# mila-iqia/babyai

Hardware: NVIDIA H100
Metric: env-steps/sec at 65 536 envs (GoToLocal); obs bit-exact vs CPU ref (higher is better)
Workload: dtype u8

## Files before the change

babyai_b200/csrc/env_logic.cuh:

```cuda
#pragma once
#include <stdint.h>

#if defined(__CUDACC__)
#define BB_HD __host__ __device__ __forceinline__
#define BB_HD_NOINLINE __host__ __device__ __noinline__
#define BB_ALIGN16 __align__(16)
#else
#define BB_ALIGN16 alignas(16)
#define BB_HD inline
#define BB_HD_NOINLINE
#endif

#ifndef BB_GEN_COOP
#define BB_GEN_COOP 1
#endif
#if defined(__CUDA_ARCH__) && BB_GEN_COOP
#define BB_GEN_WARP 1
#else
#define BB_GEN_WARP 0
#endif
#ifndef BB_GEN_OUTLINE
#define BB_GEN_OUTLINE 1
#endif
#if defined(__CUDA_ARCH__) && BB_GEN_COOP
// ... 25 lines not shown
constexpr int CELL_EMPTY = T_EMPTY;
constexpr int CELL_WALL = T_WALL | (C_GREY << 3);
constexpr int NO_OBJ = 0xFF;
constexpr int CARRY_UNTRACKED = 0x40;
constexpr int MAXUNTRACKED = 32;
constexpr int MAXOBJ = 32;
constexpr int MAXH = 25;
constexpr int MAXROOMS = 16;
constexpr int MAXTOK = 72;
constexpr int OBS_BYTES = 147;
constexpr int OBS_WORDS = 37;

enum : int {
    W_PAD = 0, W_GO, W_TO, W_PICK, W_UP, W_OPEN, W_PUT, W_NEXT, W_THE, W_A, W_OBJECT,
    W_RED, W_GREEN, W_BLUE, W_PURPLE, W_YELLOW, W_GREY,
    W_BOX, W_BALL, W_KEY, W_DOOR,
    W_IN, W_FRONT, W_OF, W_YOU, W_BEHIND, W_ON, W_YOUR, W_LEFT, W_RIGHT,
    W_THEN, W_AFTER, W_AND, W_COUNT
};

struct LevelParams {
    int32_t kind, room_size, num_rows, num_cols, num_dists, instr, doors_open, grey_dists;
    int32_t locations, unblocking, implicit_unlock;
    int32_t all_unique, require_unreachable;
    int32_t n_action_kinds, action_kinds[4];
    int32_t n_instr_kinds, instr_kinds[3];
    int32_t W, H, cells, cells_pad, max_tokens, nav_time_maze;
    int32_t strict_mask, done_actions;
    int32_t col_mul;
    int32_t kinds_mask, single_instr;
    int32_t bonus, bonus_a, bonus_b;
    int32_t box_contains;
    int32_t obj_words;
    int32_t rs_g, rs_t, gt_off;
    uint64_t locked_thr;
    uint32_t wall_rows[MAXH];
    int32_t small;
    uint64_t wall64;
    uint64_t row_tmpl[16];
};

struct BB_ALIGN16 EnvHot {
    uint8_t x, y;
    uint8_t dirflags;
    uint8_t carry;
    uint16_t step_count, max_steps;
    uint32_t cur_mask;
    uint32_t snap_mask;
};
struct BB_ALIGN16 ObjTab {
    uint8_t x[MAXOBJ], y[MAXOBJ];
    uint8_t tc[MAXOBJ];
};
struct BB_ALIGN16 InstrRec {
    uint32_t desc_mask[8];
    uint8_t leaf_kind[4];
    uint8_t leaf_pre[4];
    uint8_t root_kind;
    uint8_t side_and;
    uint8_t flags;
    uint8_t pad0;
    uint32_t pad1;
};
struct BB_ALIGN16 RngRec { uint64_t seed, draws; };

BB_HD uint32_t mulhi32(uint32_t a, uint32_t b)
// ... 2087 lines not shown
```

babyai_b200/csrc/level_params.h:

```cpp
#pragma once
#include <math.h>
#include <string.h>
#include "../../include/babyai_b200.h"
#include "env_logic.cuh"

namespace bb {

static inline const char *make_level_params(const bb_level_spec *s, LevelParams *lp)
{
    memset(lp, 0, sizeof *lp);
    if (s->kind < 0 || s->kind > 5) return "bad level kind";
    if (s->kind == BB_KIND_BONUS) { if (s->room_size < 3 || s->room_size > 20 || s->bonus < 1 || s->bonus > 20) return "bad bonus level"; }
    else if (s->room_size < 4 || s->room_size > 8) return "room_size must be in 4..8";
    if (s->num_rows < 1 || s->num_cols < 1 || s->num_rows * s->num_cols > MAXROOMS) return "too many rooms";
    lp->kind = s->kind; lp->room_size = s->room_size; lp->num_rows = s->num_rows; lp->num_cols = s->num_cols;
    lp->num_dists = s->num_dists; lp->instr = s->instr; lp->doors_open = s->doors_open; lp->grey_dists = s->grey_dists;
    lp->locations = s->locations; lp->unblocking = s->unblocking; lp->implicit_unlock = s->implicit_unlock;
    lp->all_unique = s->all_unique; lp->require_unreachable = s->require_unreachable;
    lp->strict_mask = s->strict_mask & 0x1F; lp->done_actions = s->done_actions ? 1 : 0;
    lp->kinds_mask = 0xF; lp->single_instr = 1;
    if (s->kind == BB_KIND_REDBALL || s->kind == BB_KIND_IMPUNLOCK) lp->kinds_mask = 1 << BB_I_GOTO;
    else if (s->kind == BB_KIND_OBJ) lp->kinds_mask = 1 << s->instr;
    else if (s->kind == BB_KIND_UNLOCK) lp->kinds_mask = 1 << BB_I_OPEN;
    else if (s->kind == BB_KIND_LEVELGEN) {
        lp->kinds_mask = 0;
        for (int i = 0; i < s->n_action_kinds && i < 4; i++) lp->kinds_mask |= 1 << s->action_kinds[i];
        lp->single_instr = s->n_instr_kinds == 1 && s->instr_kinds[0] == BB_K_ACTION;
    } else if (s->kind == BB_KIND_BONUS) lp->single_instr = !(s->bonus == 14 || s->bonus == 19 || s->bonus == 20);
    lp->bonus = s->kind == BB_KIND_BONUS ? s->bonus : 0; lp->bonus_a = s->bonus_a; lp->bonus_b = s->bonus_b;
    lp->box_contains = lp->bonus == BN_KEY_IN_BOX ? 2 : 0;
    if (s->kind == BB_KIND_OBJ && (s->instr < BB_I_GOTO || s->instr > BB_I_PUTNEXT)) return "bad instruction kind";
    if (s->kind == BB_KIND_OBJ && s->instr == BB_I_PUTNEXT && s->num_dists < 2) return "PutNext needs two objects";
    lp->n_action_kinds = s->n_action_kinds; lp->n_instr_kinds = s->n_instr_kinds;
    for (int i = 0; i < 4; i++) lp->action_kinds[i] = s->action_kinds[i];
    for (int i = 0; i < 3; i++) lp->instr_kinds[i] = s->instr_kinds[i];
    lp->col_mul = s->num_cols > 0 ? (64 + s->num_cols - 1) / s->num_cols : 64;
    for (int r = 0; r < s->num_rows * s->num_cols; r++)
        if (s->num_cols <= 0 || ((r * lp->col_mul) >> 6) != r / s->num_cols) return "unsupported room grid (room / num_cols by multiplication)";
    lp->W = (s->room_size - 1) * s->num_cols + 1;
    lp->H = (s->room_size - 1) * s->num_rows + 1;
    if (lp->W > MAXH || lp->H > MAXH) return "grid too large";
    lp->cells = lp->W * lp->H;
    lp->rs_g = (lp->W + 3) / 4 * 4;
    lp->rs_t = (lp->H + 3) / 4 * 4;
    lp->gt_off = (lp->H * lp->rs_g + 15) / 16 * 16;
    lp->cells_pad = lp->gt_off + (lp->W * lp->rs_t + 15) / 16 * 16;
    lp->nav_time_maze = s->room_size * s->room_size * s->num_rows * s->num_cols;
    int max_objs = s->num_dists + (s->kind == BB_KIND_OBJ ? 0 : 1);
    if (s->kind == BB_KIND_IMPUNLOCK) {
        if (s->num_rows * s->num_cols < 2) return "GoToImpUnlock needs at least two rooms";
        max_objs = s->num_dists * (s->num_rows * s->num_cols - 1) + 2;
    }
    if (s->kind == BB_KIND_UNLOCK) {
        if (s->num_rows * s->num_cols < 2) return "Unlock needs at least two rooms";
        if (s->num_dists * (s->num_rows * s->num_cols - 1) + 1 > MAXUNTRACKED) return "too many untracked objects";
        max_objs = 0;
    }
    if (s->kind == BB_KIND_LEVELGEN) {
        if (s->n_action_kinds < 1 || s->n_action_kinds > 4 || s->n_instr_kinds < 1 || s->n_instr_kinds > 3)
            return "bad LevelGen kinds";
        double t = ceil(s->locked_room_prob * 4294967296.0);
// ... 51 lines not shown
```

babyai_b200/csrc/pool.cu:

```cuda
#include <cuda_runtime.h>
#include <stdint.h>
#include <stdio.h>
#include <string.h>
#include <math.h>
#include <new>
#include <vector>
#include <stdlib.h>

#include "../../include/babyai_b200.h"
#include "env_logic.cuh"
#include "level_params.h"
#include "simt.cuh"
#include "gen_round.cuh"
#include "rollout_lane.cuh"
#include "rollout_cta.cuh"
#include "step8.cuh"
#include <type_traits>
#include "rgb_tiles.h"

using namespace bb;

struct PoolPtrs {
    uint8_t *grid; EnvHot *hot; ObjTab *obj; InstrRec *ins; int16_t *tok;
    uint8_t *rgrid; EnvHot *rhot; ObjTab *robj; InstrRec *rins; int16_t *rtok;
// ... 77 lines not shown
        const uint32_t mneed = __ballot_sync(FULL, need);
        if (mneed) {
            uint32_t base = 0;
            if (lane == 0) base = atomicAdd(P.gen_ticket, (uint32_t)__popc(mneed));
            base = __shfl_sync(FULL, base, 0);
            if (need) {
                uint32_t idx = base + (uint32_t)__popc(mneed & ((1u << lane) - 1u));
                if (idx < count) {
                    int b = 3;
                    if (idx >= c3) { idx -= c3; b = 2; if (idx >= c2) { idx -= c2; b = 1; if (idx >= c1) { idx -= c1; b = 0; } } }
                    env = P.gen_list[(size_t)b * P.n + idx];
                    tl = P.tail[env];
                    left = target - (int)(tl - P.head_snap[env]);
                    const RngRec r = P.rng[env];
                    ds.init(&s_ring[0][tid], GS_THREADS, r.seed, r.draws);
                } else exhausted = true;
            }
        }
        const bool active = left > 0;
        const uint32_t mact = __ballot_sync(FULL, active);
        if (!mact) break;
        const bool low = __any_sync(FULL, active && target - left < min_keep);
        if (max_rounds > 0 && rounds >= max_rounds && !low) break;
        if (min_active > 0 && rounds >= 1 && __popc(mact) < min_active && !low && !__any_sync(FULL, active && left > (int)(D / 2))) break;
        rounds++;
        gen_small_round<DrawRing, false>(lp, P, ds, active, env, tl, left, D);
    }
}

constexpr int R_WARPS = 2;
constexpr int R_THREADS = 32 * R_WARPS;
constexpr int R_THREADS_FUSED = R_THREADS + 32;

struct SmemOnlyMem {
    const LevelParams &lp; uint8_t *g, *o, *i;
    __device__ __forceinline__ SmemOnlyMem(const LevelParams &lp_, uint8_t *g_, uint8_t *o_, uint8_t *i_) : lp(lp_), g(g_), o(o_), i(i_) {}
    __device__ __forceinline__ int cell(int x, int y) const { return g[y * lp.rs_g + x]; }
    __device__ __forceinline__ void set_cell(int x, int y, int v) { bb::set_cell(lp, g, x, y, v); }
    __device__ __forceinline__ uint32_t word_at(int off) const { return *reinterpret_cast<const uint32_t *>(g + off); }
    __device__ __forceinline__ int ox(int k) const { return o[k]; }
    __device__ __forceinline__ int oy(int k) const { return o[MAXOBJ + k]; }
    __device__ __forceinline__ int otc(int k) const { return o[2 * MAXOBJ + k]; }
    __device__ __forceinline__ uint32_t oxw(int i) const { return reinterpret_cast<const uint32_t *>(o)[i]; }
    __device__ __forceinline__ uint32_t oyw(int i) const { return reinterpret_cast<const uint32_t *>(o)[MAXOBJ / 4 + i]; }
    __device__ __forceinline__ void set_oxy(int k, int x, int y) { o[k] = (uint8_t)x; o[MAXOBJ + k] = (uint8_t)y; }
    __device__ __forceinline__ uint32_t desc_mask(int d) const { return reinterpret_cast<const uint32_t *>(i)[d]; }
    __device__ __forceinline__ int leaf_kind(int l) const { return i[32 + l]; }
    __device__ __forceinline__ int leaf_pre(int l) const { return i[36 + l]; }
    __device__ __forceinline__ void set_leaf_pre(int l, int v) { i[36 + l] = (uint8_t)v; }
    __device__ __forceinline__ int root_kind() const { return i[40]; }
    __device__ __forceinline__ int side_and() const { return i[41]; }
    __device__ __forceinline__ void set_side_and(int v) { i[41] = (uint8_t)v; }
    __device__ __forceinline__ int flags() const { return i[42]; }
    __device__ __forceinline__ void set_flags(int v) { i[42] = (uint8_t)v; }
    __device__ __forceinline__ int start_carry() const { return i[43]; }
};

template <int K>
struct SmemRoomKindMem : SmemOnlyMem {
    static constexpr int spec_room_kinds = K;
    __device__ __forceinline__ SmemRoomKindMem(const LevelParams &lp_, uint8_t *g_, uint8_t *o_, uint8_t *i_) : SmemOnlyMem(lp_, g_, o_, i_) {}
};

template <int ACT_BYTES, bool UNTR = false, int ROOM_KINDS = 0>
__global__ void __launch_bounds__(R_THREADS_FUSED, 7)
k_rollout(const LevelParams lp, const PoolPtrs P, const void *__restrict__ actions_v, uint8_t *__restrict__ obs,
          float *__restrict__ reward, uint8_t *__restrict__ done, int8_t *__restrict__ dirs, const int n, const int T,
          const int mode, const int force_reset, const int gen_rounds, const int gen_min_active)
{
    extern __shared__ __align__(16) uint32_t smr[];
    const int lane = threadIdx.x & 31, warp = threadIdx.x >> 5;
    const int warp_words = rl_warp_words(lp);
    const bool fused = gen_rounds > 0;
    uint32_t *g_area = smr + R_WARPS * warp_words;
    volatile int *s_done = reinterpret_cast<volatile int *>(g_area + RG_AREA_WORDS - 4);
    if (warp == R_WARPS) {
        rollout_gen_warp(lp, P, g_area, s_done, n, T, blockIdx.x * R_WARPS * 32, gen_rounds, gen_min_active, lane, R_WARPS);
        return;
    }
    rollout_lane_step_warp<PoolPtrs, typename std::conditional<ROOM_KINDS != 0, SmemRoomKindMem<ROOM_KINDS>, SmemOnlyMem>::type, ACT_BYTES, UNTR>(lp, P, actions_v, obs, reward, done, dirs, n, T, mode, force_reset, fused,
                                                                   smr + warp * warp_words, lane, blockIdx.x * R_WARPS + warp, s_done);
}

template <bool UNTR>
__global__ void __launch_bounds__(RC_THREADS, 7)
k_rollout_cta(const LevelParams lp, const PoolPtrs P, const int8_t *__restrict__ actions, uint8_t *__restrict__ obs,
              float *__restrict__ reward, uint8_t *__restrict__ done, int8_t *__restrict__ dirs, const int n, const int T, const int mode)
{
    extern __shared__ __align__(16) uint32_t smc[];
    rollout_cta_role<PoolPtrs, UNTR>(lp, P, actions, obs, reward, done, dirs, n, T, mode, smc, threadIdx.x, blockIdx.x);
}
#if BB_GEN_COOP
template <bool IMPUNLOCK>
__global__ void __launch_bounds__(GEN_THREADS)
k_gen(const LevelParams lp, const PoolPtrs P, const int n, const int target, const int lanes_per_warp, const int chain_cap)
{
    __shared__ typename GenMemFor<IMPUNLOCK>::type gen_mem[GEN_THREADS / 32];
    GenMem *mem = &gen_mem[threadIdx.x >> 5];
    const int lane = threadIdx.x & 31;
    const uint32_t c3 = P.gen_count[3], c2 = P.gen_count[2], c1 = P.gen_count[1], c0 = P.gen_count[0];
    const uint32_t count = c0 + c1 + c2 + c3;
    const uint32_t D = (uint32_t)P.depth;
    for (;;) {
        uint32_t idx = 0;
        if (lane == 0) idx = atomicAdd(P.gen_ticket, 1u);
        idx = __shfl_sync(0xFFFFFFFFu, idx, 0);
        if (idx >= count) break;
        int b = 3;
        if (idx >= c3) { idx -= c3; b = 2; if (idx >= c2) { idx -= c2; b = 1; if (idx >= c1) { idx -= c1; b = 0; } } }
        const int env = P.gen_list[(size_t)b * n + idx];
        const uint32_t t0 = P.tail[env];
        const int have = (int)(t0 - P.head_snap[env]);
        int m = target - have;
// ... 483 lines not shown
    cudaStream_t st = (cudaStream_t)stream;
    if (sched_leave_rollout(p, st)) return 1;
    if (sched_before_step(p, p->rel, st)) return 1;
    launch_step(p, actions_dev, action_bytes, obs_dev, reward_dev, done_dev, dir_dev, 0, st);
    if (sched_after_step(p, p->rel, st)) return 1;
    p->rel++;
    CU(cudaGetLastError());
    return 0;
}

int bb_pool_step_timed(bb_pool *p, const void *actions_dev, int32_t action_bytes, uint8_t *obs_dev, float *reward_dev,
                       uint8_t *done_dev, int8_t *dir_dev, float *ms_step, float *ms_gen)
{
    if (!p || !actions_dev || !obs_dev || !reward_dev || !done_dev || !ms_step || !ms_gen) return fail("bad arguments");
    CU(cudaSetDevice(p->device));
    if (!p->ev[0]) for (int i = 0; i < 3; i++) CU(cudaEventCreate(&p->ev[i]));
    if (sched_join(p, p->stream)) return 1;
    p->after_rollout = false;
    launch_gen(p, p->stream);
    CU(cudaEventRecord(p->ev[0], p->stream));
    launch_step(p, actions_dev, action_bytes, obs_dev, reward_dev, done_dev, dir_dev, 0, p->stream);
    CU(cudaEventRecord(p->ev[1], p->stream));
    launch_gen(p, p->stream);
    CU(cudaEventRecord(p->ev[2], p->stream));
    CU(cudaEventSynchronize(p->ev[2]));
    CU(cudaEventElapsedTime(ms_step, p->ev[0], p->ev[1]));
    CU(cudaEventElapsedTime(ms_gen, p->ev[1], p->ev[2]));
    return 0;
}

static int rollout_graph(bb_pool *p, const int8_t *actions_dev, int32_t T, uint8_t *obs_dev, float *reward_dev,
                         uint8_t *done_dev, int8_t *dir_dev, cudaStream_t user);

int bb_pool_rollout(bb_pool *p, const int8_t *actions_dev, int32_t T, uint8_t *obs_dev, float *reward_dev,
                    uint8_t *done_dev, int8_t *dir_dev, void *stream)
{
    if (!p || !actions_dev || !obs_dev || !reward_dev || !done_dev || T < 1) return fail("bad arguments");
    BB_CHECK_RINGS(p);
    CU(cudaSetDevice(p->device));
    cudaStream_t user = (cudaStream_t)stream;
    const bool conc = p->gen_concurrent && p->mode == BB_MODE_AUTORESET;
    const bool kgen_levels = !(p->lp.small && !p->gen_generic);
    const int cap = kgen_levels && p->chain_cap > 0 && p->D >= 4 * T ? p->chain_cap : 0;
    int R = p->refill_every;
    if (conc) R = p->D / (2 * T);
    if (cap) R = p->D / (4 * T);
    if (conc || cap) { if (R > 8) R = 8; if (p->refill_cap > 0 && R > p->refill_cap) R = p->refill_cap; }
    const bool persistent = p->lp.cells_pad <= p->persist_max_cells && !p->no_persistent &&
                            (p->mode == BB_MODE_FREEZE || (conc || cap ? R >= 1 : p->D >= (p->refill_every + 1) * T));
    if (!persistent) return rollout_graph(p, actions_dev, T, obs_dev, reward_dev, done_dev, dir_dev, user);
    if (T != p->last_T) { p->rollouts = 0; p->last_T = T; }
    const bool refill_slot = (p->rollouts % R) == 0;
    if (!conc || refill_slot) { if (sched_join(p, user)) return 1; }
    const size_t smem = (size_t)R_WARPS * rl_warp_words(p->lp) * 4;
    const int blocks = (p->n + 32 * R_WARPS - 1) / (32 * R_WARPS);
    const bool fused = !p->rollout_cta && p->gen_fused != 0 && (p->gen_fused == 2 || 3 * p->lp.nav_time_maze >= 2 * T) &&
                       p->lp.small && !p->gen_generic && !p->gen_concurrent && p->mode == BB_MODE_AUTORESET &&
                       p->D >= 2 * T + 8 && !getenv("BB_DEBUG_NO_REFILL");
    if (fused && T > p->fused_T) launch_gen(p, user);
    p->fused_T = fused ? T : 0;
    const bool refill = !fused && p->mode == BB_MODE_AUTORESET && !getenv("BB_DEBUG_NO_REFILL") && refill_slot;
    p->rollouts++;
    const bool dbg_timing = p->time_rollout;
    cudaEvent_t *dbg_ev = p->tev;
    if (dbg_timing && !dbg_ev[0]) for (int i = 0; i < 4; i++) CU(cudaEventCreate(&dbg_ev[i]));
    const size_t nb = (size_t)p->n * sizeof(uint32_t);
    const bool gen_serial = !p->gen_concurrent;
    if (refill && gen_serial) {
        if (dbg_timing) cudaEventRecord(dbg_ev[2], user);
        const bool fused_snap = p->lp.small && !p->gen_generic;
        if (!fused_snap) CU(cudaMemcpyAsync(p->P.head_snap, p->P.head, nb, cudaMemcpyDeviceToDevice, user));
        launch_gen_kernel(p, p->D, user, p->gen_budget, p->gen_min_active, fused_snap, p->refill_every * T, false, cap);
        cudaMemcpyAsync(p->P.tail_pub, p->P.tail, nb, cudaMemcpyDeviceToDevice, user);
        if (dbg_timing) { cudaEventRecord(dbg_ev[3], user); p->tev_refill = true; }
        p->launches++;
    } else if (refill) {
        CU(cudaMemcpyAsync(p->P.head_snap, p->P.head, nb, cudaMemcpyDeviceToDevice, user));
        CU(cudaEventRecord(p->ev_fork, user));
    }
    if (dbg_timing) cudaEventRecord(dbg_ev[0], user);
    if (p->rollout_cta) {
        const int blocks_c = (p->n + RC_ENVS - 1) / RC_ENVS;
        const size_t smc = (size_t)rc2_cta_words(p->lp) * 4;
        if (p->lp.kind == KIND_UNLOCK) k_rollout_cta<true><<<blocks_c, RC_THREADS, smc, user>>>(p->lp, p->P, actions_dev, obs_dev, reward_dev, done_dev, dir_dev, p->n, T, p->mode);
        else k_rollout_cta<false><<<blocks_c, RC_THREADS, smc, user>>>(p->lp, p->P, actions_dev, obs_dev, reward_dev, done_dev, dir_dev, p->n, T, p->mode);
    }
    else {
        const int gr = fused ? (p->gen_budget > 0 ? p->gen_budget : 1 << 20) : 0, gm = fused ? p->gen_min_active : 0;
        const int threads = fused ? R_THREADS_FUSED : R_THREADS;
        const size_t sm = fused ? smem + RG_AREA_WORDS * 4 : smem;
#define BB_LAUNCH_ROLLOUT(...) k_rollout<__VA_ARGS__><<<blocks, threads, sm, user>>>(p->lp, p->P, actions_dev, obs_dev, reward_dev, done_dev, dir_dev, p->n, T, p->mode, 0, gr, gm)
        if (p->lp.kind == KIND_UNLOCK) BB_LAUNCH_ROLLOUT(1, true);
        else if (p->room_kinds == (1 << I_GOTO)) BB_LAUNCH_ROLLOUT(1, false, 1 << I_GOTO);
        else if (p->room_kinds == (1 << I_PICKUP)) BB_LAUNCH_ROLLOUT(1, false, 1 << I_PICKUP);
        else BB_LAUNCH_ROLLOUT(1);
#undef BB_LAUNCH_ROLLOUT
    }
    if (dbg_timing) { cudaEventRecord(dbg_ev[1], user); p->tev_kernel = true; }
    p->launches++;
    if (refill && !gen_serial) {
        CU(cudaStreamWaitEvent(p->gen_stream, p->ev_fork, 0));
        if (dbg_timing) cudaEventRecord(dbg_ev[2], p->gen_stream);
        launch_gen_kernel(p, p->D, p->gen_stream, p->gen_budget, p->gen_min_active, false, (p->refill_every + 1) * T, true, cap);
        cudaMemcpyAsync(p->P.tail_pub, p->P.tail, nb, cudaMemcpyDeviceToDevice, p->gen_stream);
        if (dbg_timing) { cudaEventRecord(dbg_ev[3], p->gen_stream); p->tev_refill = true; }
        p->gen_outstanding = true;
        p->launches++;
    }
    p->rel = 0;
    p->after_rollout = true;
    CU(cudaGetLastError());
    return 0;
}

int bb_pool_rollout_timed(bb_pool *p, const int8_t *actions_dev, int32_t T, uint8_t *obs_dev, float *reward_dev,
                          uint8_t *done_dev, int8_t *dir_dev, float *ms_rollout_kernel, float *ms_refill)
{
    if (!p || !ms_rollout_kernel || !ms_refill) return fail("bad arguments");
    *ms_rollout_kernel = 0; *ms_refill = 0;
    p->time_rollout = true; p->tev_kernel = false; p->tev_refill = false;
    const int rc = bb_pool_rollout(p, actions_dev, T, obs_dev, reward_dev, done_dev, dir_dev, p->stream);
    p->time_rollout = false;
    if (rc) return rc;
    CU(cudaStreamSynchronize(p->stream));
    CU(cudaDeviceSynchronize());
    if (p->tev[0] && p->tev_kernel) {
        CU(cudaEventElapsedTime(ms_rollout_kernel, p->tev[0], p->tev[1]));
        if (p->tev_refill) CU(cudaEventElapsedTime(ms_refill, p->tev[2], p->tev[3]));
    }
    return 0;
}

static int rollout_graph(bb_pool *p, const int8_t *actions_dev, int32_t T, uint8_t *obs_dev, float *reward_dev,
                         uint8_t *done_dev, int8_t *dir_dev, cudaStream_t user)
{
    GraphKey key = { actions_dev, obs_dev, reward_dev, done_dev, dir_dev, T, p->mode };
    if (!p->graph || memcmp(&key, &p->gkey, sizeof key) != 0) {
        if (p->graph) { cudaGraphExecDestroy(p->graph); p->graph = nullptr; }
        cudaGraph_t g;
        const size_t n = (size_t)p->n;
        const long long l0 = p->launches;
        const bool saved_out = p->gen_outstanding;
        CU(cudaStreamBeginCapture(p->stream, cudaStreamCaptureModeThreadLocal));
        p->gen_outstanding = false;
// ... 213 lines not shown
```

babyai_b200/csrc/rollout_lane.cuh:

```cuda
#pragma once
#include "simt.cuh"

namespace bb {

constexpr int RL_OBJ_STRIDE = 25, RL_INS_STRIDE = 13;
constexpr int RL_TILE_WORDS = 32 * OBS_BYTES / 4;
constexpr int R_STEP_WARPS = 2;

BB_HD int rl_warp_words(const LevelParams &lp) { return 32 * (((lp.cells_pad >> 2) | 1) + RL_OBJ_STRIDE + RL_INS_STRIDE) + RL_TILE_WORDS; }

template <bool TO_SMEM>
BB_DEV void rl_copy_records(uint32_t *sm, int stride_words, uint4 *glob, int chunks_per_env, int nv, int lane)
{
    for (int idx = lane; idx < nv * chunks_per_env; idx += 32) {
        const int e = idx / chunks_per_env, w0 = (idx - e * chunks_per_env) * 4;
        uint32_t *d = sm + e * stride_words + w0;
        if (TO_SMEM) { const uint4 v = glob[idx]; d[0] = v.x; d[1] = v.y; d[2] = v.z; d[3] = v.w; }
        else glob[idx] = make_uint4(d[0], d[1], d[2], d[3]);
    }
}

BB_DEV void rl_store_tile_plain(const uint32_t *tile, uint8_t *dst, int lane, int valid_envs)
{
    const uint8_t *s = reinterpret_cast<const uint8_t *>(tile);
    const int nbytes = valid_envs * OBS_BYTES;
    for (int i = lane; i < nbytes; i += 32) dst[i] = s[i];
}

template <class PP, class MemT, int ACT_BYTES, bool UNTR>
BB_DEV void rollout_lane_step_warp(const LevelParams &lp, const PP &P, const void *actions_v, uint8_t *obs, float *reward, uint8_t *done,
                                   int8_t *dirs, const int n, const int T, const int mode, const int force_reset, const bool fused,
                                   uint32_t *warp_smem, const int lane, const int warp_global, volatile int *s_done)
{
    const int8_t *actions = reinterpret_cast<const int8_t *>(actions_v);
    const int gs = (lp.cells_pad >> 2) | 1;
    const int env0 = warp_global * 32, env = env0 + lane;
    int nv = n - env0; nv = nv > 32 ? 32 : (nv < 0 ? 0 : nv);
    const bool valid = lane < nv;
    uint32_t *sg = warp_smem, *so = sg + 32 * gs, *si = so + 32 * RL_OBJ_STRIDE;
    uint32_t *tile = si + 32 * RL_INS_STRIDE;
    rl_copy_records<true>(sg, gs, reinterpret_cast<uint4 *>(P.grid + (size_t)env0 * lp.cells_pad), lp.cells_pad >> 4, nv, lane);
    rl_copy_records<true>(so, RL_OBJ_STRIDE, reinterpret_cast<uint4 *>(P.obj + env0), 6, nv, lane);
    rl_copy_records<true>(si, RL_INS_STRIDE, reinterpret_cast<uint4 *>(P.ins + env0), 3, nv, lane);
    EnvHot h;
    { uint4 z = make_uint4(0, 0, 0, 0); h = *reinterpret_cast<EnvHot *>(&z); }
    uint32_t head = 0, avail = 0;
    float last_rew = 0.0f;
    if (valid) {
        h = P.hot[env];
        head = P.head[env];
        avail = (fused ? P.tail[env] : BB_LDCG(P.tail_pub + env)) - head;
        if (mode == BB_MODE_FREEZE) last_rew = P.last_reward[env];
    }
    if (fused) BB_ROLE_SYNC(32 * (R_STEP_WARPS + 1));
    BB_SYNCWARP();
    MemT mem(lp, reinterpret_cast<uint8_t *>(sg + lane * gs), reinterpret_cast<uint8_t *>(so + lane * RL_OBJ_STRIDE),
             reinterpret_cast<uint8_t *>(si + lane * RL_INS_STRIDE));
    uint32_t n_step = 0, n_end = 0, n_succ = 0, n_err = 0, consumed = 0;
    const int gchunks = lp.cells_pad >> 4, tchunks = lp.max_tokens >> 3;
    const int rec_chunks = gchunks + 6 + 3;
    bool bulk_pending = false;
    int a_next = 0;
    if (valid && !force_reset) {
        if (ACT_BYTES == 1) a_next = BB_LD_S8(actions + env);
        else a_next = (int)reinterpret_cast<const long long *>(actions_v)[env];
    }
    for (int t = 0; t < T; t++) {
        const int a = a_next;
        if (ACT_BYTES == 1 && valid && t + 1 < T) a_next = BB_LD_S8(actions + (size_t)(t + 1) * n + env);
        float rew = 0.0f; bool dn = false, begin = false;
        if (valid) {
            begin = force_reset != 0;
            if (force_reset) {
            } else if (!(h.dirflags & 4)) {
                const StepResult sr = step_env<UNTR>(h, mem, a);
                rew = sr.reward; dn = sr.done;
                n_step++; n_end += dn; n_succ += sr.success;
                if (dn) {
                    if (mode == BB_MODE_AUTORESET) begin = true;
                    else { h.dirflags |= 4; last_rew = rew; }
                }
            } else { rew = last_rew; dn = true; }
            if (begin && !(consumed < avail && avail <= (uint32_t)P.depth)) { begin = false; n_err++; *P.err_flag = 1; }
        }
        uint32_t mbeg = BB_BALLOT(begin);
        if (mbeg) {
            const uint32_t my_slot = (head + consumed) % (uint32_t)P.depth;
            BB_SYNCWARP();
            while (mbeg) {
                const int src = ffs32(mbeg);
                mbeg &= mbeg - 1;
                const int slot = (int)BB_SHFL(my_slot, src);
                const int e = env0 + src;
                const LevelOut o = r2_ring_slot(lp, P, e, slot);
                for (int c = lane; c < rec_chunks + tchunks; c += 32) {
                    if (c < rec_chunks) {
                        const uint4 *sp; uint32_t *dp; int k = c;
                        if (k < gchunks) { sp = reinterpret_cast<const uint4 *>(o.grid) + k; dp = sg + src * gs + 4 * k; }
                        else if ((k -= gchunks) < 6) { sp = reinterpret_cast<const uint4 *>(o.obj) + k; dp = so + src * RL_OBJ_STRIDE + 4 * k; }
                        else { k -= 6; sp = reinterpret_cast<const uint4 *>(o.ins) + k; dp = si + src * RL_INS_STRIDE + 4 * k; }
                        const uint4 v = BB_LDCG(sp);
                        dp[0] = v.x; dp[1] = v.y; dp[2] = v.z; dp[3] = v.w;
                    } else {
                        const int k = c - rec_chunks;
                        reinterpret_cast<uint4 *>(P.tok + (size_t)e * lp.max_tokens)[k] = BB_LDCG(reinterpret_cast<const uint4 *>(o.tok) + k);
                    }
                }
                if (lane == src) {
                    const uint4 hv = BB_LDCG(reinterpret_cast<const uint4 *>(o.hot));
                    h = *reinterpret_cast<const EnvHot *>(&hv);
                    consumed++;
                }
            }
            BB_SYNCWARP();
        }
        uint32_t w[OBS_WORDS];
#pragma unroll
        for (int k = 0; k < OBS_WORDS; k++) w[k] = 0;
        if (valid) {
            if (mode == BB_MODE_AUTORESET && (int)h.step_count + 2 == (int)h.max_steps && consumed < avail) {
                const LevelOut o = r2_ring_slot(lp, P, env, (int)((head + consumed) % (uint32_t)P.depth));
                BB_PREFETCH_L2(o.grid);
                BB_PREFETCH_L2(o.obj);
                BB_PREFETCH_L2(reinterpret_cast<const uint8_t *>(o.obj) + 64);
                BB_PREFETCH_L2(o.ins);
                BB_PREFETCH_L2(reinterpret_cast<const uint8_t *>(o.ins) + 32);
                BB_PREFETCH_L2(o.hot);
                BB_PREFETCH_L2(o.tok);
            }
            observe(lp, mem, h.x, h.y, h.dirflags & 3, carry_cell_of<UNTR>(h, mem), w);
            const size_t oi = (size_t)t * n + env;
            if (reward) reward[oi] = rew;
            if (done) done[oi] = dn ? 1 : 0;
            if (dirs) dirs[oi] = (int8_t)(h.dirflags & 3);
        }
        if (lane == 0 && bulk_pending) BB_BULK_WAIT_READ();
        bulk_pending = false;
        BB_SYNCWARP();
        {
            const uint32_t next_w0 = BB_SHFL_DOWN(w[0], 1);
            stage_obs_words(tile, w, lane, next_w0);
        }
        uint8_t *dst = obs + ((size_t)t * n + env0) * OBS_BYTES;
        const bool bulk = nv == 32 && (((uintptr_t)dst) & 15) == 0;
        if (bulk) BB_FENCE_ASYNC_SMEM();
        BB_SYNCWARP();
        if (bulk) {
            if (lane == 0) { BB_BULK_STORE(dst, tile, 32 * OBS_BYTES); bulk_pending = true; }
        } else if (nv > 0) {
            rl_store_tile_plain(tile, dst, lane, nv);
            BB_SYNCWARP();
        }
    }
    if (lane == 0 && bulk_pending) BB_BULK_WAIT_READ();
    BB_SYNCWARP();
    rl_copy_records<false>(sg, gs, reinterpret_cast<uint4 *>(P.grid + (size_t)env0 * lp.cells_pad), lp.cells_pad >> 4, nv, lane);
    rl_copy_records<false>(so, RL_OBJ_STRIDE, reinterpret_cast<uint4 *>(P.obj + env0), 6, nv, lane);
    rl_copy_records<false>(si, RL_INS_STRIDE, reinterpret_cast<uint4 *>(P.ins + env0), 3, nv, lane);
    if (valid) {
        P.hot[env] = h;
        P.head[env] = head + consumed;
        if (mode == BB_MODE_FREEZE) P.last_reward[env] = last_rew;
    }
    for (int off = 16; off; off >>= 1) {
        n_step += BB_SHFL_DOWN(n_step, off); n_end += BB_SHFL_DOWN(n_end, off);
        n_succ += BB_SHFL_DOWN(n_succ, off); n_err += BB_SHFL_DOWN(n_err, off);
    }
    if (fused && lane == 0) BB_ATOMIC_ADD(const_cast<int *>(s_done), 1);
    if (lane == 0) {
        unsigned long long *c = P.warp_counters + 4ull * warp_global;
        if (n_step) BB_ATOMIC_ADD(c + 0, (unsigned long long)n_step);
        if (n_end) BB_ATOMIC_ADD(c + 1, (unsigned long long)n_end);
        if (n_succ) BB_ATOMIC_ADD(c + 2, (unsigned long long)n_succ);
        if (n_err) BB_ATOMIC_ADD(c + 3, (unsigned long long)n_err);
    }
}

}
```

babyai_b200/lib.py:

```python
import ctypes as C
import os

from .levels import LevelSpec

HERE = os.path.dirname(os.path.abspath(__file__))
LIB_PATH = os.path.join(HERE, 'libbabyai_b200.so')

SYMBOLS = [
    'bb_pool_create', 'bb_pool_destroy', 'bb_pool_seed', 'bb_pool_set_mode', 'bb_pool_reset', 'bb_pool_step',
    'bb_pool_step_timed', 'bb_pool_rollout', 'bb_pool_rollout_timed', 'bb_pool_step_host', 'bb_pool_reset_host', 'bb_pool_step_learner', 'bb_pool_mission_tokens', 'bb_pool_render_rgb', 'bb_rgb_tiles', 'bb_vocab_size',
    'bb_vocab_word', 'bb_pool_get_state', 'bb_pool_width', 'bb_pool_height', 'bb_pool_num_envs',
    'bb_pool_counters', 'bb_pool_launches', 'bb_last_error',
]

_lib = None


def load():
    global _lib
    if _lib is not None:
        return _lib
    if not os.path.exists(LIB_PATH):
        raise ImportError('%s is missing: the CUDA extension has not been built (python -m babyai_b200.build). '
                          'babyai_b200 has no CPU fallback.' % LIB_PATH)
    L = C.CDLL(LIB_PATH)
    vp, i32, i64 = C.c_void_p, C.c_int32, C.c_int64
    L.bb_pool_create.argtypes = [C.POINTER(LevelSpec), i32, i32, C.POINTER(vp)]
    L.bb_pool_destroy.argtypes = [vp]
    L.bb_pool_seed.argtypes = [vp, vp]
    L.bb_pool_set_mode.argtypes = [vp, i32]
    L.bb_pool_reset.argtypes = [vp, vp, vp, vp]
    L.bb_pool_step.argtypes = [vp, vp, i32, vp, vp, vp, vp, vp]
    L.bb_pool_step_timed.argtypes = [vp, vp, i32, vp, vp, vp, vp, C.POINTER(C.c_float), C.POINTER(C.c_float)]
    L.bb_pool_rollout.argtypes = [vp, vp, i32, vp, vp, vp, vp, vp]
    L.bb_pool_rollout_timed.argtypes = [vp, vp, i32, vp, vp, vp, vp, C.POINTER(C.c_float), C.POINTER(C.c_float)]
    L.bb_pool_step_host.argtypes = [vp, vp, vp, vp, vp, vp]
    L.bb_pool_reset_host.argtypes = [vp, vp, vp]
    L.bb_pool_step_learner.argtypes = [vp, vp, vp, vp, vp, vp, vp]
    L.bb_pool_render_rgb.argtypes = [vp, vp, vp, i32, vp]
    L.bb_rgb_tiles.argtypes = [vp]
    L.bb_pool_mission_tokens.argtypes = [vp, C.POINTER(vp), C.POINTER(i32)]
    L.bb_vocab_size.restype = i32
    L.bb_vocab_word.restype = C.c_char_p
    L.bb_vocab_word.argtypes = [i32]
    L.bb_pool_get_state.argtypes = [vp, i32, vp, vp]
    L.bb_pool_width.argtypes = [vp]
    L.bb_pool_height.argtypes = [vp]
    L.bb_pool_num_envs.argtypes = [vp]
    L.bb_pool_counters.argtypes = [vp, vp]
    L.bb_pool_launches.restype = i64
    L.bb_pool_launches.argtypes = [vp]
    L.bb_last_error.restype = C.c_char_p
    _lib = L
    return L


def check(rc):
    if rc != 0:
        raise RuntimeError('babyai_b200: ' + load().bb_last_error().decode())
```

include/babyai_b200.h:

```cpp
#ifndef BABYAI_B200_H
#define BABYAI_B200_H

#include <stdint.h>

#ifdef __cplusplus
extern "C" {
#endif

#define BB_OBS_BYTES 147
#define BB_MAX_OBJ 32
#define BB_MAX_TOKENS 72

#define BB_KIND_REDBALL 0
#define BB_KIND_OBJ 1
#define BB_KIND_LEVELGEN 2
#define BB_KIND_IMPUNLOCK 3
#define BB_KIND_UNLOCK 4
#define BB_KIND_BONUS 5
#define BB_I_GOTO 0
#define BB_I_PICKUP 1
#define BB_I_OPEN 2
#define BB_I_PUTNEXT 3
#define BB_K_ACTION 0
#define BB_K_AND 1
// ... 14 lines not shown
    int32_t strict_mask;
    int32_t done_actions;
    int32_t bonus, bonus_a, bonus_b;
} bb_level_spec;

typedef struct bb_pool bb_pool;

#define BB_MODE_AUTORESET 0
#define BB_MODE_FREEZE 1

int bb_pool_create(const bb_level_spec *spec, int32_t n_envs, int32_t device, bb_pool **out);
int bb_pool_destroy(bb_pool *pool);

int bb_pool_seed(bb_pool *pool, const uint64_t *seeds_host);

int bb_pool_set_mode(bb_pool *pool, int32_t mode);

int bb_pool_reset(bb_pool *pool, uint8_t *obs_dev, int8_t *dir_dev, void *stream);

int bb_pool_step(bb_pool *pool, const void *actions_dev, int32_t action_bytes,
                 uint8_t *obs_dev, float *reward_dev, uint8_t *done_dev, int8_t *dir_dev, void *stream);

int bb_pool_step_timed(bb_pool *pool, const void *actions_dev, int32_t action_bytes,
                       uint8_t *obs_dev, float *reward_dev, uint8_t *done_dev, int8_t *dir_dev,
                       float *ms_step_kernel, float *ms_gen_kernel);

int bb_pool_rollout(bb_pool *pool, const int8_t *actions_dev, int32_t T,
                    uint8_t *obs_dev, float *reward_dev, uint8_t *done_dev, int8_t *dir_dev, void *stream);

int bb_pool_rollout_timed(bb_pool *pool, const int8_t *actions_dev, int32_t T,
                          uint8_t *obs_dev, float *reward_dev, uint8_t *done_dev, int8_t *dir_dev,
                          float *ms_rollout_kernel, float *ms_refill);

int bb_pool_step_host(bb_pool *pool, const int8_t *actions_host,
                      uint8_t *obs_host, float *reward_host, uint8_t *done_host, int8_t *dir_host);
int bb_pool_reset_host(bb_pool *pool, uint8_t *obs_host, int8_t *dir_host);

int bb_pool_step_learner(bb_pool *pool, const int8_t *actions_host, uint8_t *obs_dev, float *reward_host,
                         uint8_t *done_host, int8_t *dir_dev, void *stream);

int bb_pool_render_rgb(bb_pool *pool, const uint8_t *obs_dev, uint8_t *rgb_dev, int32_t n_obs, void *stream);
int bb_rgb_tiles(uint8_t *tiles_host);

int bb_pool_mission_tokens(bb_pool *pool, const int16_t **tokens_dev, int32_t *max_len);
int32_t bb_vocab_size(void);
const char *bb_vocab_word(int32_t id);

int bb_pool_get_state(bb_pool *pool, int32_t env, uint8_t *grid_host, int32_t *info_host);
int32_t bb_pool_width(const bb_pool *pool);
int32_t bb_pool_height(const bb_pool *pool);
int32_t bb_pool_num_envs(const bb_pool *pool);

int bb_pool_counters(bb_pool *pool, int64_t *out4_host);

int64_t bb_pool_launches(const bb_pool *pool);

const char *bb_last_error(void);

#ifdef __cplusplus
}
#endif
#endif
```

Before: 7.574 billion.

## Pack per-lane object and instruction records compactly in shared memory

Replaces the fixed-stride object and instruction shared-memory tables with one compact per-lane record. Its size follows the level's object count and description words, and objects are laid out interleaved. This shrinks rollout shared memory per warp, and the launch bound is raised from 7 to 8 blocks per SM to use the freed space. For room-kind-specialised kernels it also ignores force_reset, and it adds a query that reports occupancy. The cost is more complex gather/scatter index math when copying records and refilling slots.

```diff
diff --git a/babyai_b200/csrc/env_logic.cuh b/babyai_b200/csrc/env_logic.cuh
--- a/babyai_b200/csrc/env_logic.cuh
+++ b/babyai_b200/csrc/env_logic.cuh
@@ -81,6 +81,7 @@
     int32_t bonus, bonus_a, bonus_b;
     int32_t box_contains;
     int32_t obj_words;
+    int32_t desc_words;
     int32_t rs_g, rs_t, gt_off;
     uint64_t locked_thr;
     uint32_t wall_rows[MAXH];
diff --git a/babyai_b200/csrc/level_params.h b/babyai_b200/csrc/level_params.h
--- a/babyai_b200/csrc/level_params.h
+++ b/babyai_b200/csrc/level_params.h
@@ -27,6 +27,7 @@
         for (int i = 0; i < s->n_action_kinds && i < 4; i++) lp->kinds_mask |= 1 << s->action_kinds[i];
         lp->single_instr = s->n_instr_kinds == 1 && s->instr_kinds[0] == BB_K_ACTION;
     } else if (s->kind == BB_KIND_BONUS) lp->single_instr = !(s->bonus == 14 || s->bonus == 19 || s->bonus == 20);
+    lp->desc_words = lp->single_instr ? 2 : 8;
     lp->bonus = s->kind == BB_KIND_BONUS ? s->bonus : 0; lp->bonus_a = s->bonus_a; lp->bonus_b = s->bonus_b;
     lp->box_contains = lp->bonus == BN_KEY_IN_BOX ? 2 : 0;
     if (s->kind == BB_KIND_OBJ && (s->instr < BB_I_GOTO || s->instr > BB_I_PUTNEXT)) return "bad instruction kind";
diff --git a/babyai_b200/csrc/pool.cu b/babyai_b200/csrc/pool.cu
--- a/babyai_b200/csrc/pool.cu
+++ b/babyai_b200/csrc/pool.cu
@@ -133,38 +133,8 @@
 constexpr int R_THREADS = 32 * R_WARPS;
 constexpr int R_THREADS_FUSED = R_THREADS + 32;
 
-struct SmemOnlyMem {
-    const LevelParams &lp; uint8_t *g, *o, *i;
-    __device__ __forceinline__ SmemOnlyMem(const LevelParams &lp_, uint8_t *g_, uint8_t *o_, uint8_t *i_) : lp(lp_), g(g_), o(o_), i(i_) {}
-    __device__ __forceinline__ int cell(int x, int y) const { return g[y * lp.rs_g + x]; }
-    __device__ __forceinline__ void set_cell(int x, int y, int v) { bb::set_cell(lp, g, x, y, v); }
-    __device__ __forceinline__ uint32_t word_at(int off) const { return *reinterpret_cast<const uint32_t *>(g + off); }
-    __device__ __forceinline__ int ox(int k) const { return o[k]; }
-    __device__ __forceinline__ int oy(int k) const { return o[MAXOBJ + k]; }
-    __device__ __forceinline__ int otc(int k) const { return o[2 * MAXOBJ + k]; }
-    __device__ __forceinline__ uint32_t oxw(int i) const { return reinterpret_cast<const uint32_t *>(o)[i]; }
-    __device__ __forceinline__ uint32_t oyw(int i) const { return reinterpret_cast<const uint32_t *>(o)[MAXOBJ / 4 + i]; }
-    __device__ __forceinline__ void set_oxy(int k, int x, int y) { o[k] = (uint8_t)x; o[MAXOBJ + k] = (uint8_t)y; }
-    __device__ __forceinline__ uint32_t desc_mask(int d) const { return reinterpret_cast<const uint32_t *>(i)[d]; }
-    __device__ __forceinline__ int leaf_kind(int l) const { return i[32 + l]; }
-    __device__ __forceinline__ int leaf_pre(int l) const { return i[36 + l]; }
-    __device__ __forceinline__ void set_leaf_pre(int l, int v) { i[36 + l] = (uint8_t)v; }
-    __device__ __forceinline__ int root_kind() const { return i[40]; }
-    __device__ __forceinline__ int side_and() const { return i[41]; }
-    __device__ __forceinline__ void set_side_and(int v) { i[41] = (uint8_t)v; }
-    __device__ __forceinline__ int flags() const { return i[42]; }
-    __device__ __forceinline__ void set_flags(int v) { i[42] = (uint8_t)v; }
-    __device__ __forceinline__ int start_carry() const { return i[43]; }
-};
-
-template <int K>
-struct SmemRoomKindMem : SmemOnlyMem {
-    static constexpr int spec_room_kinds = K;
-    __device__ __forceinline__ SmemRoomKindMem(const LevelParams &lp_, uint8_t *g_, uint8_t *o_, uint8_t *i_) : SmemOnlyMem(lp_, g_, o_, i_) {}
-};
-
 template <int ACT_BYTES, bool UNTR = false, int ROOM_KINDS = 0>
-__global__ void __launch_bounds__(R_THREADS_FUSED, 7)
+__global__ void __launch_bounds__(R_THREADS_FUSED, 8)
 k_rollout(const LevelParams lp, const PoolPtrs P, const void *__restrict__ actions_v, uint8_t *__restrict__ obs,
           float *__restrict__ reward, uint8_t *__restrict__ done, int8_t *__restrict__ dirs, const int n, const int T,
           const int mode, const int force_reset, const int gen_rounds, const int gen_min_active)
@@ -179,7 +149,7 @@
         rollout_gen_warp(lp, P, g_area, s_done, n, T, blockIdx.x * R_WARPS * 32, gen_rounds, gen_min_active, lane, R_WARPS);
         return;
     }
-    rollout_lane_step_warp<PoolPtrs, typename std::conditional<ROOM_KINDS != 0, SmemRoomKindMem<ROOM_KINDS>, SmemOnlyMem>::type, ACT_BYTES, UNTR>(lp, P, actions_v, obs, reward, done, dirs, n, T, mode, force_reset, fused,
+    rollout_lane_step_warp<PoolPtrs, LaneRecMem<ROOM_KINDS>, ACT_BYTES, UNTR>(lp, P, actions_v, obs, reward, done, dirs, n, T, mode, ROOM_KINDS != 0 ? 0 : force_reset, fused,
                                                                    smr + warp * warp_words, lane, blockIdx.x * R_WARPS + warp, s_done);
 }
 
@@ -729,6 +699,22 @@
 static int rollout_graph(bb_pool *p, const int8_t *actions_dev, int32_t T, uint8_t *obs_dev, float *reward_dev,
                          uint8_t *done_dev, int8_t *dir_dev, cudaStream_t user);
 
+static bool rollout_fused(const bb_pool *p, int T)
+{
+    return !p->rollout_cta && p->gen_fused != 0 && (p->gen_fused == 2 || 3 * p->lp.nav_time_maze >= 2 * T) &&
+           p->lp.small && !p->gen_generic && !p->gen_concurrent && p->mode == BB_MODE_AUTORESET &&
+           p->D >= 2 * T + 8 && !getenv("BB_DEBUG_NO_REFILL");
+}
+
+using RolloutKernel = decltype(&k_rollout<1>);
+static RolloutKernel rollout_kernel(const bb_pool *p)
+{
+    if (p->lp.kind == KIND_UNLOCK) return k_rollout<1, true>;
+    if (p->room_kinds == (1 << I_GOTO)) return k_rollout<1, false, 1 << I_GOTO>;
+    if (p->room_kinds == (1 << I_PICKUP)) return k_rollout<1, false, 1 << I_PICKUP>;
+    return k_rollout<1>;
+}
+
 int bb_pool_rollout(bb_pool *p, const int8_t *actions_dev, int32_t T, uint8_t *obs_dev, float *reward_dev,
                     uint8_t *done_dev, int8_t *dir_dev, void *stream)
 {
@@ -751,9 +737,7 @@
     if (!conc || refill_slot) { if (sched_join(p, user)) return 1; }
     const size_t smem = (size_t)R_WARPS * rl_warp_words(p->lp) * 4;
     const int blocks = (p->n + 32 * R_WARPS - 1) / (32 * R_WARPS);
-    const bool fused = !p->rollout_cta && p->gen_fused != 0 && (p->gen_fused == 2 || 3 * p->lp.nav_time_maze >= 2 * T) &&
-                       p->lp.small && !p->gen_generic && !p->gen_concurrent && p->mode == BB_MODE_AUTORESET &&
-                       p->D >= 2 * T + 8 && !getenv("BB_DEBUG_NO_REFILL");
+    const bool fused = rollout_fused(p, T);
     if (fused && T > p->fused_T) launch_gen(p, user);
     p->fused_T = fused ? T : 0;
     const bool refill = !fused && p->mode == BB_MODE_AUTORESET && !getenv("BB_DEBUG_NO_REFILL") && refill_slot;
@@ -786,12 +770,7 @@
         const int gr = fused ? (p->gen_budget > 0 ? p->gen_budget : 1 << 20) : 0, gm = fused ? p->gen_min_active : 0;
         const int threads = fused ? R_THREADS_FUSED : R_THREADS;
         const size_t sm = fused ? smem + RG_AREA_WORDS * 4 : smem;
-#define BB_LAUNCH_ROLLOUT(...) k_rollout<__VA_ARGS__><<<blocks, threads, sm, user>>>(p->lp, p->P, actions_dev, obs_dev, reward_dev, done_dev, dir_dev, p->n, T, p->mode, 0, gr, gm)
-        if (p->lp.kind == KIND_UNLOCK) BB_LAUNCH_ROLLOUT(1, true);
-        else if (p->room_kinds == (1 << I_GOTO)) BB_LAUNCH_ROLLOUT(1, false, 1 << I_GOTO);
-        else if (p->room_kinds == (1 << I_PICKUP)) BB_LAUNCH_ROLLOUT(1, false, 1 << I_PICKUP);
-        else BB_LAUNCH_ROLLOUT(1);
-#undef BB_LAUNCH_ROLLOUT
+        rollout_kernel(p)<<<blocks, threads, sm, user>>>(p->lp, p->P, actions_dev, obs_dev, reward_dev, done_dev, dir_dev, p->n, T, p->mode, 0, gr, gm);
     }
     if (dbg_timing) { cudaEventRecord(dbg_ev[1], user); p->tev_kernel = true; }
     p->launches++;
@@ -807,6 +786,28 @@
     p->rel = 0;
     p->after_rollout = true;
     CU(cudaGetLastError());
+    return 0;
+}
+
+int bb_pool_rollout_residency(bb_pool *p, int32_t T, int32_t *ctas_per_sm, int32_t *ctas, int32_t *sms)
+{
+    if (!p || T < 1 || !ctas_per_sm || !ctas || !sms) return fail("bad arguments");
+    CU(cudaSetDevice(p->device));
+    const void *fn; int threads; size_t smem;
+    if (p->rollout_cta) {
+        fn = p->lp.kind == KIND_UNLOCK ? (const void *)k_rollout_cta<true> : (const void *)k_rollout_cta<false>;
+        threads = RC_THREADS; smem = (size_t)rc2_cta_words(p->lp) * 4;
+        *ctas = (p->n + RC_ENVS - 1) / RC_ENVS;
+    } else {
+        const bool fused = rollout_fused(p, T);
+        fn = (const void *)rollout_kernel(p);
+        threads = fused ? R_THREADS_FUSED : R_THREADS;
+        smem = (size_t)R_WARPS * rl_warp_words(p->lp) * 4 + (fused ? RG_AREA_WORDS * 4 : 0);
+        *ctas = (p->n + 32 * R_WARPS - 1) / (32 * R_WARPS);
+    }
+    int per_sm = 0;
+    CU(cudaOccupancyMaxActiveBlocksPerMultiprocessor(&per_sm, fn, threads, smem));
+    *ctas_per_sm = per_sm; *sms = p->sm_count;
     return 0;
 }
 
diff --git a/babyai_b200/csrc/rollout_lane.cuh b/babyai_b200/csrc/rollout_lane.cuh
--- a/babyai_b200/csrc/rollout_lane.cuh
+++ b/babyai_b200/csrc/rollout_lane.cuh
@@ -3,11 +3,56 @@
 
 namespace bb {
 
-constexpr int RL_OBJ_STRIDE = 25, RL_INS_STRIDE = 13;
 constexpr int RL_TILE_WORDS = 32 * OBS_BYTES / 4;
 constexpr int R_STEP_WARPS = 2;
 
-BB_HD int rl_warp_words(const LevelParams &lp) { return 32 * (((lp.cells_pad >> 2) | 1) + RL_OBJ_STRIDE + RL_INS_STRIDE) + RL_TILE_WORDS; }
+BB_HD int rl_rec_words(const LevelParams &lp) { return 4 + 3 * lp.obj_words + lp.desc_words; }
+BB_HD int rl_rec_stride(const LevelParams &lp) { return rl_rec_words(lp) | 1; }
+BB_HD int rl_obj_byte(int k) { return 16 + k + ((k >> 2) << 3); }
+BB_HD int rl_mask_byte(const LevelParams &lp, int d) { return 16 + 12 * lp.obj_words + 4 * d; }
+constexpr int RL_CHUNKS = (int)(sizeof(ObjTab) + sizeof(InstrRec)) / 16;
+BB_HD int rl_chunk_word(const LevelParams &lp, int c, int q)
+{
+    if (c < 6) { const int w = 4 * c + q, g = w & 7; return g < lp.obj_words ? 4 + 3 * g + (w >> 3) : -1; }
+    const int w = 4 * (c - 6) + q;
+    return w >= 8 ? w - 8 : (w < lp.desc_words ? 4 + 3 * lp.obj_words + w : -1);
+}
+BB_HD uint32_t *rl_rec_src(const LevelParams &lp, ObjTab *obj, InstrRec *ins, int j)
+{
+    uint32_t *o = reinterpret_cast<uint32_t *>(obj), *i = reinterpret_cast<uint32_t *>(ins);
+    const int ow = 3 * lp.obj_words;
+    if (j < 4) return i + 8 + j;
+    if ((j -= 4) < ow) return o + (j % 3) * (MAXOBJ / 4) + j / 3;
+    return i + (j - ow);
+}
+
+template <int K>
+struct LaneRecMem {
+    static constexpr int spec_room_kinds = K;
+    const LevelParams &lp; uint8_t *g, *r;
+    BB_HD LaneRecMem(const LevelParams &lp_, uint8_t *g_, uint8_t *r_) : lp(lp_), g(g_), r(r_) {}
+    BB_HD int cell(int x, int y) const { return g[y * lp.rs_g + x]; }
+    BB_HD void set_cell(int x, int y, int v) { bb::set_cell(lp, g, x, y, v); }
+    BB_HD uint32_t word_at(int off) const { return load_u32_any(g + off); }
+    BB_HD int ox(int k) const { return r[rl_obj_byte(k)]; }
+    BB_HD int oy(int k) const { return r[rl_obj_byte(k) + 4]; }
+    BB_HD int otc(int k) const { return r[rl_obj_byte(k) + 8]; }
+    BB_HD uint32_t oxw(int i) const { return load_u32_any(r + rl_obj_byte(4 * i)); }
+    BB_HD uint32_t oyw(int i) const { return load_u32_any(r + rl_obj_byte(4 * i) + 4); }
+    BB_HD void set_oxy(int k, int x, int y) { r[rl_obj_byte(k)] = (uint8_t)x; r[rl_obj_byte(k) + 4] = (uint8_t)y; }
+    BB_HD uint32_t desc_mask(int d) const { return load_u32_any(r + rl_mask_byte(lp, d)); }
+    BB_HD int leaf_kind(int l) const { return r[l]; }
+    BB_HD int leaf_pre(int l) const { return r[4 + l]; }
+    BB_HD void set_leaf_pre(int l, int v) { r[4 + l] = (uint8_t)v; }
+    BB_HD int root_kind() const { return r[8]; }
+    BB_HD int side_and() const { return r[9]; }
+    BB_HD void set_side_and(int v) { r[9] = (uint8_t)v; }
+    BB_HD int flags() const { return r[10]; }
+    BB_HD void set_flags(int v) { r[10] = (uint8_t)v; }
+    BB_HD int start_carry() const { return r[11]; }
+};
+
+BB_HD int rl_warp_words(const LevelParams &lp) { return 32 * (((lp.cells_pad >> 2) | 1) + rl_rec_stride(lp)) + RL_TILE_WORDS; }
 
 template <bool TO_SMEM>
 BB_DEV void rl_copy_records(uint32_t *sm, int stride_words, uint4 *glob, int chunks_per_env, int nv, int lane)
@@ -20,6 +65,36 @@
     }
 }
 
+template <bool TO_SMEM>
+BB_DEV void rl_copy_recs(const LevelParams &lp, uint32_t *sr, int rs, ObjTab *obj, InstrRec *ins, int nv, int lane)
+{
+    constexpr int EPP = 32 / RL_CHUNKS;
+    const int c = lane % RL_CHUNKS;
+    int r[4];
+#pragma unroll
+    for (int q = 0; q < 4; q++) r[q] = rl_chunk_word(lp, c, q);
+    if (lane >= EPP * RL_CHUNKS || r[0] < 0) return;
+#pragma unroll 4
+    for (int e = lane / RL_CHUNKS; e < nv; e += EPP) {
+        uint32_t *rec = sr + e * rs;
+        uint4 *g = c < 6 ? reinterpret_cast<uint4 *>(obj + e) + c : reinterpret_cast<uint4 *>(ins + e) + (c - 6);
+        if (TO_SMEM) {
+            const uint4 v = *g;
+            rec[r[0]] = v.x;
+            if (r[1] >= 0) rec[r[1]] = v.y;
+            if (r[2] >= 0) rec[r[2]] = v.z;
+            if (r[3] >= 0) rec[r[3]] = v.w;
+        } else if (r[3] >= 0) {
+            *g = make_uint4(rec[r[0]], rec[r[1]], rec[r[2]], rec[r[3]]);
+        } else {
+            uint32_t *gw = reinterpret_cast<uint32_t *>(g);
+            gw[0] = rec[r[0]];
+            if (r[1] >= 0) gw[1] = rec[r[1]];
+            if (r[2] >= 0) gw[2] = rec[r[2]];
+        }
+    }
+}
+
 BB_DEV void rl_store_tile_plain(const uint32_t *tile, uint8_t *dst, int lane, int valid_envs)
 {
     const uint8_t *s = reinterpret_cast<const uint8_t *>(tile);
@@ -37,11 +112,11 @@
     const int env0 = warp_global * 32, env = env0 + lane;
     int nv = n - env0; nv = nv > 32 ? 32 : (nv < 0 ? 0 : nv);
     const bool valid = lane < nv;
-    uint32_t *sg = warp_smem, *so = sg + 32 * gs, *si = so + 32 * RL_OBJ_STRIDE;
-    uint32_t *tile = si + 32 * RL_INS_STRIDE;
+    const int rs = rl_rec_stride(lp);
+    uint32_t *sg = warp_smem, *sr = sg + 32 * gs;
+    uint32_t *tile = sr + 32 * rs;
     rl_copy_records<true>(sg, gs, reinterpret_cast<uint4 *>(P.grid + (size_t)env0 * lp.cells_pad), lp.cells_pad >> 4, nv, lane);
-    rl_copy_records<true>(so, RL_OBJ_STRIDE, reinterpret_cast<uint4 *>(P.obj + env0), 6, nv, lane);
-    rl_copy_records<true>(si, RL_INS_STRIDE, reinterpret_cast<uint4 *>(P.ins + env0), 3, nv, lane);
+    rl_copy_recs<true>(lp, sr, rs, P.obj + env0, P.ins + env0, nv, lane);
     EnvHot h;
     { uint4 z = make_uint4(0, 0, 0, 0); h = *reinterpret_cast<EnvHot *>(&z); }
     uint32_t head = 0, avail = 0;
@@ -54,11 +129,9 @@
     }
     if (fused) BB_ROLE_SYNC(32 * (R_STEP_WARPS + 1));
     BB_SYNCWARP();
-    MemT mem(lp, reinterpret_cast<uint8_t *>(sg + lane * gs), reinterpret_cast<uint8_t *>(so + lane * RL_OBJ_STRIDE),
-             reinterpret_cast<uint8_t *>(si + lane * RL_INS_STRIDE));
+    LaneRecMem<mem_spec<MemT>::room_kinds> mem(lp, reinterpret_cast<uint8_t *>(sg + lane * gs), reinterpret_cast<uint8_t *>(sr + lane * rs));
     uint32_t n_step = 0, n_end = 0, n_succ = 0, n_err = 0, consumed = 0;
     const int gchunks = lp.cells_pad >> 4, tchunks = lp.max_tokens >> 3;
-    const int rec_chunks = gchunks + 6 + 3;
     bool bulk_pending = false;
     int a_next = 0;
     if (valid && !force_reset) {
@@ -86,6 +159,7 @@
         uint32_t mbeg = BB_BALLOT(begin);
         if (mbeg) {
             const uint32_t my_slot = (head + consumed) % (uint32_t)P.depth;
+            const int rec_items = gchunks + rl_rec_words(lp);
             BB_SYNCWARP();
             while (mbeg) {
                 const int src = ffs32(mbeg);
@@ -93,16 +167,16 @@
                 const int slot = (int)BB_SHFL(my_slot, src);
                 const int e = env0 + src;
                 const LevelOut o = r2_ring_slot(lp, P, e, slot);
-                for (int c = lane; c < rec_chunks + tchunks; c += 32) {
-                    if (c < rec_chunks) {
-                        const uint4 *sp; uint32_t *dp; int k = c;
-                        if (k < gchunks) { sp = reinterpret_cast<const uint4 *>(o.grid) + k; dp = sg + src * gs + 4 * k; }
-                        else if ((k -= gchunks) < 6) { sp = reinterpret_cast<const uint4 *>(o.obj) + k; dp = so + src * RL_OBJ_STRIDE + 4 * k; }
-                        else { k -= 6; sp = reinterpret_cast<const uint4 *>(o.ins) + k; dp = si + src * RL_INS_STRIDE + 4 * k; }
-                        const uint4 v = BB_LDCG(sp);
+                for (int c = lane; c < rec_items + tchunks; c += 32) {
+                    if (c < gchunks) {
+                        const uint4 v = BB_LDCG(reinterpret_cast<const uint4 *>(o.grid) + c);
+                        uint32_t *dp = sg + src * gs + 4 * c;
                         dp[0] = v.x; dp[1] = v.y; dp[2] = v.z; dp[3] = v.w;
+                    } else if (c < rec_items) {
+                        const int k = c - gchunks;
+                        sr[src * rs + k] = BB_LDCG(rl_rec_src(lp, o.obj, o.ins, k));
                     } else {
-                        const int k = c - rec_chunks;
+                        const int k = c - rec_items;
                         reinterpret_cast<uint4 *>(P.tok + (size_t)e * lp.max_tokens)[k] = BB_LDCG(reinterpret_cast<const uint4 *>(o.tok) + k);
                     }
                 }
@@ -155,8 +229,7 @@
     if (lane == 0 && bulk_pending) BB_BULK_WAIT_READ();
     BB_SYNCWARP();
     rl_copy_records<false>(sg, gs, reinterpret_cast<uint4 *>(P.grid + (size_t)env0 * lp.cells_pad), lp.cells_pad >> 4, nv, lane);
-    rl_copy_records<false>(so, RL_OBJ_STRIDE, reinterpret_cast<uint4 *>(P.obj + env0), 6, nv, lane);
-    rl_copy_records<false>(si, RL_INS_STRIDE, reinterpret_cast<uint4 *>(P.ins + env0), 3, nv, lane);
+    rl_copy_recs<false>(lp, sr, rs, P.obj + env0, P.ins + env0, nv, lane);
     if (valid) {
         P.hot[env] = h;
         P.head[env] = head + consumed;
diff --git a/babyai_b200/lib.py b/babyai_b200/lib.py
--- a/babyai_b200/lib.py
+++ b/babyai_b200/lib.py
@@ -8,7 +8,7 @@
 
 SYMBOLS = [
     'bb_pool_create', 'bb_pool_destroy', 'bb_pool_seed', 'bb_pool_set_mode', 'bb_pool_reset', 'bb_pool_step',
-    'bb_pool_step_timed', 'bb_pool_rollout', 'bb_pool_rollout_timed', 'bb_pool_step_host', 'bb_pool_reset_host', 'bb_pool_step_learner', 'bb_pool_mission_tokens', 'bb_pool_render_rgb', 'bb_rgb_tiles', 'bb_vocab_size',
+    'bb_pool_step_timed', 'bb_pool_rollout', 'bb_pool_rollout_timed', 'bb_pool_rollout_residency', 'bb_pool_step_host', 'bb_pool_reset_host', 'bb_pool_step_learner', 'bb_pool_mission_tokens', 'bb_pool_render_rgb', 'bb_rgb_tiles', 'bb_vocab_size',
     'bb_vocab_word', 'bb_pool_get_state', 'bb_pool_width', 'bb_pool_height', 'bb_pool_num_envs',
     'bb_pool_counters', 'bb_pool_launches', 'bb_last_error',
 ]
@@ -34,6 +34,7 @@
     L.bb_pool_step_timed.argtypes = [vp, vp, i32, vp, vp, vp, vp, C.POINTER(C.c_float), C.POINTER(C.c_float)]
     L.bb_pool_rollout.argtypes = [vp, vp, i32, vp, vp, vp, vp, vp]
     L.bb_pool_rollout_timed.argtypes = [vp, vp, i32, vp, vp, vp, vp, C.POINTER(C.c_float), C.POINTER(C.c_float)]
+    L.bb_pool_rollout_residency.argtypes = [vp, i32, C.POINTER(i32), C.POINTER(i32), C.POINTER(i32)]
     L.bb_pool_step_host.argtypes = [vp, vp, vp, vp, vp, vp]
     L.bb_pool_reset_host.argtypes = [vp, vp, vp]
     L.bb_pool_step_learner.argtypes = [vp, vp, vp, vp, vp, vp, vp]
diff --git a/include/babyai_b200.h b/include/babyai_b200.h
--- a/include/babyai_b200.h
+++ b/include/babyai_b200.h
@@ -70,6 +70,8 @@
                           uint8_t *obs_dev, float *reward_dev, uint8_t *done_dev, int8_t *dir_dev,
                           float *ms_rollout_kernel, float *ms_refill);
 
+int bb_pool_rollout_residency(bb_pool *pool, int32_t T, int32_t *ctas_per_sm, int32_t *ctas, int32_t *sms);
+
 int bb_pool_step_host(bb_pool *pool, const int8_t *actions_host,
                       uint8_t *obs_host, float *reward_host, uint8_t *done_host, int8_t *dir_host);
 int bb_pool_reset_host(bb_pool *pool, uint8_t *obs_host, int8_t *dir_host);
```

After: 8.458 billion (median of 6 runs). 1.12x the previous value.
